# nianticlabs/simplerecon

Hardware: AMD Instinct MI355X
Metric: depth frames/sec (640x480, 7 src views, 64 planes) (higher is better)
Workload: dtype f32

## Files before the change

### include/simplerecon_hip.h

```cpp
#ifndef SIMPLERECON_HIP_H_
#define SIMPLERECON_HIP_H_

#include <stddef.h>
#include <stdint.h>

#ifdef __cplusplus
extern "C" {
#endif

#define SR_OK 0
#define SR_ERR_INVALID_ARGUMENT 1
#define SR_ERR_UNSUPPORTED 2
#define SR_ERR_WORKSPACE_TOO_SMALL 3
#define SR_ERR_HIP_BASE 1000

enum {
  SR_OPT_MLP_SPLIT = 0, SR_OPT_WINO_SPLIT, SR_OPT_WINO_XCD, SR_OPT_WINO_NT, SR_OPT_WINO_KSPLIT, SR_OPT_CONV_WINO,
  SR_OPT_CONV_TILE, SR_OPT_CONV_KSPLIT, SR_OPT_PW_NT, SR_OPT_PW_KS, SR_OPT_PT_CFG, SR_OPT_PT_KS, SR_OPT_DOT_LDS,
  SR_OPT_DOT_LDS_G, SR_OPT_DOT_LDS_CULL, SR_OPT_DOT_LDS_CAP, SR_OPT_UPSAMPLE_QUAD, SR_OPT_POOL_STREAM,
  SR_OPT_MLP_TILE,
  SR_OPT_COUNT
};
int sr_option_count(void);
const char* sr_option_name(int id);
int sr_option_id(const char* name);
int sr_option_get(int id, int* value);
int sr_option_set(int id, int value, int* previous );
int sr_option_default(int id, int* value);

int sr_abi_version(void);

const char* sr_target_arch(void);


size_t sr_volume_workspace_bytes(int B, int K, int C, int h, int w);

int sr_volume_prepare(const float* src, const float* K_src, const float* T_src_cur,
                      const float* T_cur_src, int B, int K, int C, int h, int w, void* workspace,
                      size_t workspace_bytes, void* stream);

int sr_dot_volume_sweep(const float* cur, const float* invK_cur, const float* planes, int64_t ps_b,
                        int64_t ps_d, int64_t ps_y, int64_t ps_x, int B, int K, int C, int h, int w,
                        int D, float* out_cv, int64_t cv_sb, int64_t cv_sd, int64_t cv_sp,
                        float* out_lowest, uint8_t* out_mask, void* workspace,
                        size_t workspace_bytes, void* stream);

int sr_conv3x3_wino_io_nhwc_fwd(const void* in, int64_t in_batch_stride, int in_pix_stride, const float* packed_u,
                                const float* bias, const void* residual, int64_t res_batch_stride, int res_pix_stride,
                                void* out, int64_t out_batch_stride, int out_pix_stride, int B, int H, int W, int Cin,
                                int Cout, float leaky_slope, int io_dtype, void* stream);
int sr_pw_conv_io_nhwc_fwd(const void* in, int64_t in_batch_stride, int in_pix_stride, const float* packed_w,
                           const float* bias, const void* residual, int64_t res_batch_stride, int res_pix_stride, void* out,
                           int64_t out_batch_stride, int out_pix_stride, int B, int HW, int Cin, int Cout, float act_code,
                           int io_dtype, void* stream);

size_t sr_pw_conv_tiled_workspace_bytes(int M, int Cin, int Cout);
int sr_pw_conv_tiled_plan(int M, int Cin, int Cout, int can_split, int* cfg, int* ks);
int sr_pw_conv_tiled_nhwc_fwd(const float* in, int in_pix_stride, const float* packed_w, const float* bias,
                              const float* gate, const float* residual, int res_pix_stride, float* out,
                              int out_pix_stride, int M, int HW, int Cin, int Cout, float act_code, void* workspace,
                              size_t workspace_bytes, void* stream);
int sr_pw_conv_supported(int Cin, int Cout);
int sr_pw_conv_plan(int B, int HW, int Cin, int Cout, int* nt, int* ks);
int sr_pw_conv_nhwc_fwd(const float* in, int64_t in_batch_stride, int in_pix_stride, const float* packed_w,
                        const float* bias, const float* gate, const float* residual, int64_t res_batch_stride,
                        int res_pix_stride, float* out, int64_t out_batch_stride, int out_pix_stride, int B, int HW,
                        int Cin, int Cout, float act_code, void* stream);

int sr_backproject_fwd(const float* depth, const float* invK, float* out_points, int B, int h, int w, void* stream);
int sr_project3d_fwd(const float* points, const float* K, const float* T, float* out, int B, int N, float eps,
                     void* stream);
int sr_backproject_bwd(const float* grad_points, const float* invK, float* grad_depth, int B, int h, int w, void* stream);
int sr_project3d_bwd(const float* grad_out, const float* points, const float* K, const float* T, float* grad_points, int B,
// ... 508 lines not shown
```

### simplerecon_amd/csrc/sr_common.h

```cpp
#pragma once
#include <hip/hip_runtime.h>
#include <stdint.h>

#include "simplerecon_hip.h"

#define SR_GEOM_STRIDE 20

#define SR_WAVE 64

int sr_opt(int id);

int sr_device_cus();

hipError_t sr_allow_lds(const void* kernel, size_t bytes);

enum SrKernel { SR_K_NONE = 0, SR_K_CONV, SR_K_WINO, SR_K_WINO_SPLIT, SR_K_WINO4, SR_K_PW, SR_K_PW_TILED, SR_K_STEM, SR_K_C1S,
                SR_K_T16 };
struct SrLaunchNote { int kernel, a, b, c, d, e, f; int64_t m, n, k; };
void sr_note_launch(const SrLaunchNote& note);

int sr_wgrad_reduce_launch(const float* part, float* d_weight, int Cout, int Cin, int taps, int ci_blocks, int per, int blocks,
                           hipStream_t stream);
int sr_bias_partial_reduce_launch(const float* partial, int blocks, int C, float* d_bias, hipStream_t stream);

static inline int sr_hip_rc(hipError_t e) { return e == hipSuccess ? SR_OK : SR_ERR_HIP_BASE + (int)e; }

static inline size_t sr_align_up(size_t v, size_t a) { return (v + a - 1) / a * a; }

struct SrPlanes {
  const float* ptr;
  int64_t sb, sd, sy, sx;
};

struct SrVolumeOut {
  float* cv;
  int64_t sb, sd, sp;
  float* lowest;
  uint8_t* mask;
};

struct SrSample {
  float zp;
  float pix_x, pix_y;
  float w_nw, w_ne, w_sw, w_se;
  int o_nw, o_ne, o_sw, o_se;
  bool any_tap;
};

typedef float sr_f2v __attribute__((ext_vector_type(2)));
typedef float f32x16 __attribute__((ext_vector_type(16)));

__device__ __forceinline__ void sr_bilinear_taps(float ix, float iy, int h, int w, float& fx0, float& fy0, float& w_nw,
                                                 float& w_ne, float& w_sw, float& w_se, bool& any_tap) {
#pragma clang fp contract(off)
  const sr_f2v ixy = {ix, iy};
  fx0 = floorf(ix);
  fy0 = floorf(iy);
  const sr_f2v f0 = {fx0, fy0};
  const sr_f2v f1 = f0 + 1.0f;
  const float fx1 = f1.x, fy1 = f1.y;
  const float wm = (float)(w - 1), hm = (float)(h - 1);
  const bool vx0 = (fx0 >= 0.0f) & (fx0 <= wm), vx1 = (fx1 >= 0.0f) & (fx1 <= wm);
  const bool vy0 = (fy0 >= 0.0f) & (fy0 <= hm), vy1 = (fy1 >= 0.0f) & (fy1 <= hm);
  const sr_f2v a1 = f1 - ixy, a0 = ixy - f0;
  const sr_f2v wtop = sr_f2v{a1.x, a0.x} * a1.y;
  const sr_f2v wbot = sr_f2v{a1.x, a0.x} * a0.y;
  w_nw = (vx0 & vy0) ? wtop.x : 0.0f;
  w_ne = (vx1 & vy0) ? wtop.y : 0.0f;
  w_sw = (vx0 & vy1) ? wbot.x : 0.0f;
  w_se = (vx1 & vy1) ? wbot.y : 0.0f;
  any_tap = (vx0 | vx1) & (vy0 | vy1);
}
__device__ __forceinline__ void sr_bilinear_taps(float ix, float iy, int h, int w, float& fx0, float& fy0, float& w_nw,
                                                 float& w_ne, float& w_sw, float& w_se) {
  bool any_tap;
  sr_bilinear_taps(ix, iy, h, w, fx0, fy0, w_nw, w_ne, w_sw, w_se, any_tap);
}

struct SrSampleXY {
  float zp, pix_x, pix_y;
// ... 114 lines not shown
__device__ __forceinline__ SrDotLane sr_dot_lane(const SrDotParams& p, int grp, int S) {
  SrDotLane l;
  l.lane = threadIdx.x & 63;
  l.grp = grp;
  l.S = S;
  l.b = blockIdx.y;
  l.N = p.h * p.w;
  l.tile = blockIdx.x;
  {
    const int nwg = gridDim.x, q = nwg >> 3, r = nwg & 7, xcd = l.tile & 7, idx = l.tile >> 3;
    l.tile = (xcd < r ? xcd * (q + 1) : r * (q + 1) + (xcd - r) * q) + idx;
  }
  l.pix = l.tile * 64 + l.lane;
  l.active = l.pix < l.N;
  l.pc = l.active ? l.pix : l.N - 1;
  l.y = l.pc / p.w;
  l.x = l.pc - l.y * p.w;
  const int per = (p.D + l.S - 1) / l.S;
  l.j0 = l.grp * per;
  l.j1 = min(p.D, l.j0 + per);
  return l;
}
__device__ __forceinline__ void sr_argmax_step(float cost, float d, float& best, float& best_d, bool& have) {
  if (!have || cost > best || (cost != cost && best == best)) { best = cost; best_d = d; have = true; }
}
__device__ __forceinline__ void sr_dot_store_lowest(const SrDotParams& p, const SrDotLane& l, float* smem, float best,
                                                    float best_d, bool have) {
  if (p.out.lowest) {
    if (gridDim.z > 1) {
    } else if (l.S == 1) {
      if (l.active) p.out.lowest[(size_t)l.b * l.N + l.pix] = best_d;
    } else {
      float* s_best = smem;
      float* s_d = smem + l.S * 64;
      float* s_have = smem + 2 * l.S * 64;
      s_best[l.grp * 64 + l.lane] = best;
      s_d[l.grp * 64 + l.lane] = best_d;
      s_have[l.grp * 64 + l.lane] = have ? 1.0f : 0.0f;
      __syncthreads();
      if (l.grp == 0 && l.active) {
        float bb = best, bd = best_d;
        for (int g = 1; g < l.S; ++g)
          if (s_have[g * 64 + l.lane] != 0.0f &&
              (s_best[g * 64 + l.lane] > bb || (s_best[g * 64 + l.lane] != s_best[g * 64 + l.lane] && bb == bb))) {
            bb = s_best[g * 64 + l.lane];
            bd = s_d[g * 64 + l.lane];
          }
        p.out.lowest[(size_t)l.b * l.N + l.pix] = bd;
      }
    }
  }
}

static inline float* sr_ws_geom(void* workspace) { return (float*)sr_align_up((size_t)workspace, 256); }
static inline float* sr_ws_src_nhwc(void* workspace, int B, int K) {
  return (float*)((char*)sr_ws_geom(workspace) + sr_align_up((size_t)B * K * SR_GEOM_STRIDE * sizeof(float), 256));
}

static inline size_t sr_ws_nhwc_bytes(int B, int K, int C, int h, int w) {
  return sr_align_up((size_t)B * K * h * w * C * sizeof(float), 256);
}
static inline unsigned long long* sr_ws_keys(void* workspace, int B, int K, int C, int h, int w) {
  return (unsigned long long*)((char*)sr_ws_src_nhwc(workspace, B, K) + sr_ws_nhwc_bytes(B, K, C, h, w));
}

int sr_launch_dot_volume_lds(const SrDotParams& p, unsigned long long* keys, hipStream_t stream);
int sr_launch_geom(const float* K_src, const float* T_src_cur, const float* T_cur_src, float* geom,
                   int n, hipStream_t stream);
int sr_launch_argmax_planes(const float* cv, int64_t sb, int64_t sd, int64_t sp, SrPlanes planes, int B, int h, int w,
                            int D, float* lowest, hipStream_t stream);
int sr_launch_splitk_reduce(const float* part, int ksplit, int64_t part_stride, const float* bias, const float* res,
                            int64_t res_sb, int res_sp, float* out, int64_t out_sb, int out_sp, int B, int HW, int Cout,
                            float slope, hipStream_t stream);
int sr_launch_unpack_nhwc(const float* src_nhwc, float* dst_nchw, int images, int C, int npix, hipStream_t stream);
int sr_launch_pack_nhwc(const float* src_nchw, float* dst_nhwc, int images, int C, int npix,
                        hipStream_t stream);
```

### simplerecon_amd/csrc/sr_dot_volume.hip

```cpp
#include <stdlib.h>

#include "sr_common.h"


__global__ void sr_geom_kernel(const float* __restrict__ K_src, const float* __restrict__ T_src_cur,
                               const float* __restrict__ T_cur_src, float* __restrict__ geom, int n) {
#pragma clang fp contract(off)
  const int i = blockIdx.x * blockDim.x + threadIdx.x;
  if (i >= n) return;
  const float* Km = K_src + 16 * (size_t)i;
  const float* T = T_src_cur + 16 * (size_t)i;
  float* g = geom + SR_GEOM_STRIDE * (size_t)i;
  for (int r = 0; r < 3; ++r)
    for (int c = 0; c < 4; ++c) {
      float s = 0.0f;
      for (int k = 0; k < 4; ++k) s += Km[r * 4 + k] * T[k * 4 + c];
      g[r * 4 + c] = s;
    }
  float t0 = 0.f, t1 = 0.f, t2 = 0.f, dist = 0.f, rm = 0.f, tm = 0.f;
  if (T_cur_src) {
    const float* Tc = T_cur_src + 16 * (size_t)i;
    t0 = Tc[3]; t1 = Tc[7]; t2 = Tc[11];
    const float tr = (Tc[0] + Tc[5]) + Tc[10];
    const float trc = tr > 3.0f ? 3.0f : tr;
    rm = sqrtf(2.0f * (1.0f - trc / 3.0f));
    tm = sqrtf((t0 * t0 + t1 * t1) + t2 * t2);
    dist = sqrtf(tm * tm + rm * rm);
  }
  g[12] = t0; g[13] = t1; g[14] = t2; g[15] = dist; g[16] = rm; g[17] = tm; g[18] = 0.f; g[19] = 0.f;
}

int sr_launch_geom(const float* K_src, const float* T_src_cur, const float* T_cur_src, float* geom,
                   int n, hipStream_t stream) {
  if (n == 0) return SR_OK;
  hipLaunchKernelGGL(sr_geom_kernel, dim3((n + 63) / 64), dim3(64), 0, stream, K_src, T_src_cur, T_cur_src,
                     geom, n);
  return sr_hip_rc(hipGetLastError());
}

template <int C>
__global__ __launch_bounds__(256) void sr_pack_nhwc_kernel(const float* __restrict__ src,
                                                           float* __restrict__ dst, int npix) {
  __shared__ float tile[64][C + 1];
  const int img = blockIdx.y;
  const int p0 = blockIdx.x * 64;
  const float* s = src + (size_t)img * C * npix;
  float* d = dst + (size_t)img * npix * C;
  for (int e = threadIdx.x; e < 64 * C; e += 256) {
    const int c = e >> 6, p = e & 63;
    tile[p][c] = (p0 + p < npix) ? s[(size_t)c * npix + p0 + p] : 0.0f;
  }
  __syncthreads();
  for (int e = threadIdx.x; e < 64 * C; e += 256) {
    const int p = e / C, c = e - p * C;
    if (p0 + p < npix) d[(size_t)(p0 + p) * C + c] = tile[p][c];
  }
}

int sr_launch_pack_nhwc(const float* src_nchw, float* dst_nhwc, int images, int C, int npix,
                        hipStream_t stream) {
  if (images == 0 || npix == 0) return SR_OK;
// ... 130 lines not shown
#pragma unroll 1
    for (int k = 0; k < p.K; ++k) {
      SrSample s;
      sr_project_sample(geom_b + k * SR_GEOM_STRIDE, X0, X1, X2, p.h, p.w, p.inv_w, p.inv_h, s);
      const bool front = s.zp > 0.0f;
      any_depth |= front;
      any_bounds |= sr_in_bounds(s, p.h, p.w);
      const float w_nw = front ? s.w_nw : 0.0f, w_ne = front ? s.w_ne : 0.0f;
      const float w_sw = front ? s.w_sw : 0.0f, w_se = front ? s.w_se : 0.0f;
      const float* img = src_b + (size_t)k * N * C + 4 * quad;
#pragma unroll
      for (int r = 0; r < 4; ++r) {
        const int sl = 16 * r + slot;
        const int o_nw = __shfl(s.o_nw, sl), o_ne = __shfl(s.o_ne, sl), o_sw = __shfl(s.o_sw, sl), o_se = __shfl(s.o_se, sl);
        const float a_nw = __shfl(w_nw, sl), a_ne = __shfl(w_ne, sl), a_sw = __shfl(w_sw, sl), a_se = __shfl(w_se, sl);
        const float4 t_nw = *reinterpret_cast<const float4*>(img + (size_t)o_nw * C);
        const float4 t_ne = *reinterpret_cast<const float4*>(img + (size_t)o_ne * C);
        const float4 t_sw = *reinterpret_cast<const float4*>(img + (size_t)o_sw * C);
        const float4 t_se = *reinterpret_cast<const float4*>(img + (size_t)o_se * C);
        const sr_f2 cl = {curq[r].x, curq[r].y}, ch = {curq[r].z, curq[r].w};
        const sr_f2 wnw = {a_nw, a_nw}, wne = {a_ne, a_ne}, wsw = {a_sw, a_sw}, wse = {a_se, a_se};
        sr_f2 lo = wnw * sr_f2{t_nw.x, t_nw.y}, hi = wnw * sr_f2{t_nw.z, t_nw.w};
        lo = __builtin_elementwise_fma(wne, sr_f2{t_ne.x, t_ne.y}, lo);
        hi = __builtin_elementwise_fma(wne, sr_f2{t_ne.z, t_ne.w}, hi);
        lo = __builtin_elementwise_fma(wsw, sr_f2{t_sw.x, t_sw.y}, lo);
        hi = __builtin_elementwise_fma(wsw, sr_f2{t_sw.z, t_sw.w}, hi);
        lo = __builtin_elementwise_fma(wse, sr_f2{t_se.x, t_se.y}, lo);
        hi = __builtin_elementwise_fma(wse, sr_f2{t_se.z, t_se.w}, hi);
        const sr_f2 pr = __builtin_elementwise_fma(hi, ch, lo * cl);
        costr[r] += pr.x + pr.y;
      }
    }
    float cost = 0.0f;
#pragma unroll
    for (int r = 0; r < 4; ++r) {
      const float v = __shfl(sr_quad_sum(costr[r]), gather_lane);
      cost = (lane >> 4) == r ? v : cost;
    }
    if (active) out[j * p.out.sd] = cost;
    sr_argmax_step(cost, d, best, best_d, have);
    if (j == p.D - 1 && p.out.mask && active)
      p.out.mask[(size_t)b * N + pix] = (uint8_t)(any_depth && any_bounds);
  }

  sr_dot_store_lowest(p, l, smem, best, best_d, have);
}


extern "C" int sr_abi_version(void) { return 4; }
extern "C" const char* sr_target_arch(void) { return "gfx950"; }

extern "C" size_t sr_volume_workspace_bytes(int B, int K, int C, int h, int w) {
  if (B < 0 || K < 0 || C < 0 || h < 0 || w < 0) return 0;
  const size_t geom = sr_align_up((size_t)B * K * SR_GEOM_STRIDE * sizeof(float), 256);
  const size_t nhwc = sr_ws_nhwc_bytes(B, K, C, h, w);
  const size_t keys = sr_align_up((size_t)B * h * w * sizeof(unsigned long long), 256);
  return geom + nhwc + keys + 256;
}

static int sr_pick_plane_split(int B, int N, int D) {
  const long tiles = (long)B * ((N + 63) / 64);
  int S = 1;
  while (S < 16 && tiles * S < 256L * 16 && S * 2 <= D) S *= 2;
  return S;
}

extern "C" int sr_volume_prepare(const float* src, const float* K_src, const float* T_src_cur,
                                 const float* T_cur_src, int B, int K, int C, int h, int w, void* workspace,
                                 size_t workspace_bytes, void* stream_) {
  if (B < 0 || K <= 0 || C <= 0 || h <= 0 || w <= 0) return SR_ERR_INVALID_ARGUMENT;
  if (B == 0) return SR_OK;
  if (!src || !K_src || !T_src_cur || !workspace) return SR_ERR_INVALID_ARGUMENT;
  if (C % 4 != 0 || C > 32) return SR_ERR_UNSUPPORTED;
  if (workspace_bytes < sr_volume_workspace_bytes(B, K, C, h, w)) return SR_ERR_WORKSPACE_TOO_SMALL;
  hipStream_t stream = (hipStream_t)stream_;
  int rc = sr_launch_geom(K_src, T_src_cur, T_cur_src, sr_ws_geom(workspace), B * K, stream);
  if (rc) return rc;
  return sr_launch_pack_nhwc(src, sr_ws_src_nhwc(workspace, B, K), B * K, C, h * w, stream);
}

extern "C" int sr_dot_volume_sweep(const float* cur, const float* invK_cur, const float* planes, int64_t ps_b,
                                   int64_t ps_d, int64_t ps_y, int64_t ps_x, int B, int K, int C, int h, int w,
                                   int D, float* out_cv, int64_t cv_sb, int64_t cv_sd, int64_t cv_sp,
                                   float* out_lowest, uint8_t* out_mask, void* workspace,
                                   size_t workspace_bytes, void* stream_) {
  if (B < 0 || K <= 0 || C <= 0 || h <= 0 || w <= 0 || D <= 0) return SR_ERR_INVALID_ARGUMENT;
  if (B == 0) return SR_OK;
  if (!cur || !invK_cur || !planes || !out_cv || !workspace) return SR_ERR_INVALID_ARGUMENT;
  if (C % 4 != 0 || C > 32) return SR_ERR_UNSUPPORTED;
  if (workspace_bytes < sr_volume_workspace_bytes(B, K, C, h, w)) return SR_ERR_WORKSPACE_TOO_SMALL;
  hipStream_t stream = (hipStream_t)stream_;
  const int N = h * w;

  SrDotParams p;
  p.cur = cur; p.src_nhwc = sr_ws_src_nhwc(workspace, B, K); p.invK = invK_cur; p.geom = sr_ws_geom(workspace);
  p.planes = {planes, ps_b, ps_d, ps_y, ps_x};
  p.out = {out_cv, cv_sb, cv_sd, cv_sp, out_lowest, out_mask};
  p.B = B; p.K = K; p.h = h; p.w = w; p.D = D;
  p.inv_w = (float)(1.0 / (double)w);
  p.inv_h = (float)(1.0 / (double)h);

  if (C == 16) {
    const int use_lds = sr_opt(SR_OPT_DOT_LDS);
    if (use_lds) {
      const int rc = sr_launch_dot_volume_lds(p, sr_ws_keys(workspace, B, K, C, h, w), stream);
      if (rc != SR_ERR_UNSUPPORTED) return rc;
    }
// ... 108 lines not shown
```

### simplerecon_amd/csrc/sr_mlp_volume.hip

```cpp
#include <stdlib.h>
#include <string.h>

#include "sr_buffer.h"
#include "sr_view.h"

#define SR_HID 128
#define SR_VIEW_SLOTS 24
#define SR_INV_FIXED 20
#define SR_PLANE_CHUNK 8

static inline int sr_mlp_steps_var(int K) { return (SR_VIEW_SLOTS / 2) * K; }
static inline int sr_mlp_steps_inv(int K) { return (SR_INV_FIXED + 3 * K + 1) / 2; }
static inline int sr_mlp_steps1(int K) { return sr_mlp_steps_var(K) + sr_mlp_steps_inv(K); }
#define SR_MLP_STEPS2 65

static inline size_t sr_mlp_packed_floats(int K) { return (size_t)(sr_mlp_steps1(K) + SR_MLP_STEPS2) * 256 + 128 + 4; }

#define SR_MLP_COLUMN_OFFSETS(K, C)                                                                    \
  const int o_cur = (K) * (C), o_mask = o_cur + (C), o_z = o_mask + (K), o_d = o_z + (K), o_dot = o_d + 1; \
  const int o_ang = o_dot + (K), o_cray = o_ang + (K), o_sray = o_cray + 3, o_pd = o_sray + 3 * (K);  \
  const int o_rm = o_pd + (K), o_tm = o_rm + (K);
__device__ __forceinline__ int sr_mlp_var_col(int K, int C, int k, int s) {
  SR_MLP_COLUMN_OFFSETS(K, C)
  (void)o_cur; (void)o_cray; (void)o_pd; (void)o_rm; (void)o_tm;
  if (s < 16) return k * C + s;
  if (s == 16) return o_mask + k;
  if (s == 17) return o_z + k;
  if (s == 18) return o_ang + k;
  if (s < 22) return o_sray + 3 * k + (s - 19);
  if (s == 22) return o_dot + k;
  return (k == 0) ? o_d : -1;
}
__device__ __forceinline__ int sr_mlp_inv_col(int K, int C, int u) {
  SR_MLP_COLUMN_OFFSETS(K, C)
  (void)o_mask; (void)o_z; (void)o_d; (void)o_dot; (void)o_ang; (void)o_sray;
  if (u < 16) return o_cur + u;
  if (u < 19) return o_cray + (u - 16);
  if (u == 19) return -2;
  if (u >= SR_INV_FIXED + 3 * K) return -1;
  const int k = (u - SR_INV_FIXED) / 3, i = (u - SR_INV_FIXED) - 3 * k;
  return (i == 0 ? o_pd : (i == 1 ? o_rm : o_tm)) + k;
}

__global__ void sr_mlp_pack_kernel(const float* __restrict__ W1, const float* __restrict__ b1,
                                   const float* __restrict__ W2, const float* __restrict__ b2,
                                   const float* __restrict__ W3, const float* __restrict__ b3,
                                   float* __restrict__ packed, int K, int C) {
  const int steps_var = (SR_VIEW_SLOTS / 2) * K;
  const int steps1 = steps_var + (SR_INV_FIXED + 3 * K + 1) / 2;
  const int Cin = C * (K + 1) + 10 * K + 4;
  const int total = (steps1 + SR_MLP_STEPS2) * 256 + 128 + 1;
  for (int e = blockIdx.x * blockDim.x + threadIdx.x; e < total; e += gridDim.x * blockDim.x) {
    float v = 0.0f;
    if (e < steps1 * 256) {
      const int t = e >> 8, lane = (e >> 2) & 63, mt = e & 3;
      const int row = 32 * mt + (lane & 31);
      int col;
      if (t < steps_var) {
        const int slot = 2 * t + (lane >> 5);
        const int k = slot / SR_VIEW_SLOTS;
        col = sr_mlp_var_col(K, C, k, slot - k * SR_VIEW_SLOTS);
      } else {
        col = sr_mlp_inv_col(K, C, 2 * (t - steps_var) + (lane >> 5));
      }
      v = (col >= 0) ? W1[(size_t)row * Cin + col] : (col == -2 ? b1[row] : 0.0f);
    } else if (e < (steps1 + SR_MLP_STEPS2) * 256) {
      const int e2 = e - steps1 * 256;
      const int t = e2 >> 8, lane = (e2 >> 2) & 63, mt = e2 & 3;
      const int row = 32 * mt + (lane & 31);
      if (t < 64) {
        const int m = t >> 4, r = t & 15;
        const int f = 32 * m + (r & 3) + 8 * (r >> 2) + 4 * (lane >> 5);
        v = W2[(size_t)row * SR_HID + f];
      } else {
        v = (lane < 32) ? b2[row] : 0.0f;
      }
    } else if (e < (steps1 + SR_MLP_STEPS2) * 256 + 128) {
      const int i = e - (steps1 + SR_MLP_STEPS2) * 256;
      const int half = i >> 6, mt = (i >> 4) & 3, r = i & 15;
      v = W3[32 * mt + (r & 3) + 8 * (r >> 2) + 4 * half];
    } else {
      v = b3[0];
    }
    packed[e] = v;
  }
}


struct SrMlpParams {
  const float* cur;
  const float* src_nhwc;
  const float* invK;
  const float* geom;
  const float* packed;
  SrPlanes planes;
  SrVolumeOut out;
  int B, K, h, w, D;
  int tiles;
  int tiles_x;
  int th_log2, tw_log2;
  int chunk, chunks;
  int cur_nhwc;
  int vec_store;
  float inv_w, inv_h, slope;
};

__device__ __forceinline__ bool sr_mlp_lane_pixel(const SrMlpParams& p, int tile, int lane, int& y, int& x) {
  if (p.tiles_x) {
    const int ty = tile / p.tiles_x, tx = tile - ty * p.tiles_x;
    const int ly = (ty << p.th_log2) + (lane >> p.tw_log2);
    const int lx = (tx << p.tw_log2) + (lane & ((1 << p.tw_log2) - 1));
    y = min(ly, p.h - 1);
    x = min(lx, p.w - 1);
    return ly < p.h && lx < p.w;
  }
  const int N = p.h * p.w, pix = tile * 64 + lane;
  const int pc = min(pix, N - 1);
  y = pc / p.w;
  x = pc - y * p.w;
  return pix < N;
}

__device__ __forceinline__ void sr_swap_halves(float fa, float fb, float& bP, float& bQ) {
  auto r = __builtin_amdgcn_permlane32_swap(__float_as_uint(fa), __float_as_uint(fb), false, false);
  bP = __uint_as_float(r[0]);
  bQ = __uint_as_float(r[1]);
}

#define SR_MFMA(a, b, c) __builtin_amdgcn_mfma_f32_32x32x2f32((a), (b), (c), 0, 0, 0)

__device__ __forceinline__ void sr_l1_step(f32x16 (&acc)[2][4], const float4 wA, float fa, float fb) {
  float bP, bQ;
  sr_swap_halves(fa, fb, bP, bQ);
  acc[0][0] = SR_MFMA(wA.x, bP, acc[0][0]);
  acc[1][0] = SR_MFMA(wA.x, bQ, acc[1][0]);
  acc[0][1] = SR_MFMA(wA.y, bP, acc[0][1]);
  acc[1][1] = SR_MFMA(wA.y, bQ, acc[1][1]);
  acc[0][2] = SR_MFMA(wA.z, bP, acc[0][2]);
  acc[1][2] = SR_MFMA(wA.z, bQ, acc[1][2]);
  acc[0][3] = SR_MFMA(wA.w, bP, acc[0][3]);
  acc[1][3] = SR_MFMA(wA.w, bQ, acc[1][3]);
}

__device__ __forceinline__ void sr_l1_step_init(f32x16 (&acc)[2][4], const f32x16 (&hc)[2][4], const float4 wA,
                                                float fa, float fb) {
  float bP, bQ;
  sr_swap_halves(fa, fb, bP, bQ);
  acc[0][0] = SR_MFMA(wA.x, bP, hc[0][0]);
  acc[1][0] = SR_MFMA(wA.x, bQ, hc[1][0]);
  acc[0][1] = SR_MFMA(wA.y, bP, hc[0][1]);
  acc[1][1] = SR_MFMA(wA.y, bQ, hc[1][1]);
  acc[0][2] = SR_MFMA(wA.z, bP, hc[0][2]);
  acc[1][2] = SR_MFMA(wA.z, bQ, hc[1][2]);
  acc[0][3] = SR_MFMA(wA.w, bP, hc[0][3]);
  acc[1][3] = SR_MFMA(wA.w, bQ, hc[1][3]);
}

__device__ __forceinline__ int sr_opaque(bool flag) {
  int v = __builtin_amdgcn_readfirstlane((int)flag);
  asm volatile("" : "+s"(v));
  return v;
}

#define SR_LDS_W3_FLOATS 256


__device__ __forceinline__ void sr_mlp_cur_ray(float d0, float r0, float r1, float r2, float& cr0, float& cr1, float& cr2,
                                               float& crn0, float& crn1, float& crn2) {
#pragma clang fp contract(off)
  const float X0 = d0 * r0, X1 = d0 * r1, X2 = d0 * r2;
  const float cden = fmaxf(sqrtf((X0 * X0 + X1 * X1) + X2 * X2), 1e-12f);
  cr0 = X0 / cden; cr1 = X1 / cden; cr2 = X2 / cden;
  const float n1 = fmaxf(sqrtf((cr0 * cr0 + cr1 * cr1) + cr2 * cr2), 1e-5f);
  crn0 = cr0 / n1; crn1 = cr1 / n1; crn2 = cr2 / n1;
}

__device__ __forceinline__ void sr_mlp_load_taps(const float* img, const SrSample& smp, float4 (&taps)[16]) {
  const float4* t_nw = reinterpret_cast<const float4*>(img + (size_t)smp.o_nw * 16);
  const float4* t_ne = reinterpret_cast<const float4*>(img + (size_t)smp.o_ne * 16);
  const float4* t_sw = reinterpret_cast<const float4*>(img + (size_t)smp.o_sw * 16);
  const float4* t_se = reinterpret_cast<const float4*>(img + (size_t)smp.o_se * 16);
#pragma unroll
  for (int i = 0; i < 4; ++i) {
    taps[i] = t_nw[i]; taps[4 + i] = t_ne[i]; taps[8 + i] = t_sw[i]; taps[12 + i] = t_se[i];
  }
}

template <bool W1_LDS, bool W2_LDS>
__global__ __launch_bounds__(256, 1) void sr_mlp_volume_kernel(SrMlpParams p) {
  extern __shared__ __attribute__((aligned(16))) float lds[];
  constexpr int C = 16;
  constexpr int VS = SR_VIEW_SLOTS / 2;
  const int lane = threadIdx.x & 63;
  const int steps_var = VS * p.K;
  const int steps1 = steps_var + (SR_INV_FIXED + 3 * p.K + 1) / 2;
  const float4* gW1 = reinterpret_cast<const float4*>(p.packed);
  const float4* gW1inv = gW1 + (size_t)steps_var * 64;
  const float4* gW2 = gW1 + (size_t)steps1 * 64;
  const float* gW3 = p.packed + (size_t)(steps1 + SR_MLP_STEPS2) * 256;

  for (int i = threadIdx.x; i < 129; i += blockDim.x) lds[i] = gW3[i];
  constexpr int W2_FLOATS = W2_LDS ? SR_MLP_STEPS2 * 256 : 0;
  if (W2_LDS) {
    float4* l4 = reinterpret_cast<float4*>(lds + SR_LDS_W3_FLOATS);
    for (int i = threadIdx.x; i < SR_MLP_STEPS2 * 64; i += blockDim.x) l4[i] = gW2[i];
  }
  if (W1_LDS) {
    float4* l4 = reinterpret_cast<float4*>(lds + SR_LDS_W3_FLOATS + W2_FLOATS);
    for (int i = threadIdx.x; i < steps_var * 64; i += blockDim.x) l4[i] = gW1[i];
  }
  __syncthreads();
  const float4* W1p = W1_LDS ? reinterpret_cast<const float4*>(lds + SR_LDS_W3_FLOATS + W2_FLOATS) : gW1;

  const int N = p.h * p.w;
  const long nunits = (long)p.B * p.tiles * p.chunks;
  constexpr int WPB = 4;
  const int wid = __builtin_amdgcn_readfirstlane(threadIdx.x >> 6);
  long wave0 = (long)blockIdx.x * WPB + wid;
  long nwaves = (long)gridDim.x * WPB;
  long unit_end = nunits;
  if ((gridDim.x & 7) == 0) {
    const long u8 = (nunits + 7) / 8;
    const int xcd = blockIdx.x & 7;
    nwaves = (long)(gridDim.x >> 3) * WPB;
    wave0 = xcd * u8 + (long)(blockIdx.x >> 3) * WPB + wid;
    unit_end = min(nunits, (xcd + 1) * u8);
  }
  const int half = lane >> 5;

  const int rot = (int)max(1L, nwaves / p.chunks);
  for (long unit = wave0; unit < unit_end; unit += nwaves) {
    const long tb = unit / p.chunks;
    const int chunk = (int)((unit % p.chunks + tb / rot) % p.chunks);
    const int tile = (int)(tb % p.tiles);
    const int b = (int)(tb / p.tiles);
    const int j0 = chunk * p.chunk, j1 = min(p.D, j0 + p.chunk);
    int y, x;
    const bool in_image = sr_mlp_lane_pixel(p, tile, lane, y, x);
    const int pc = y * p.w + x;
    const int pix = in_image ? pc : -1;
    const bool active = pix >= 0;
    const float* plane_ptr = p.planes.ptr + b * p.planes.sb + y * p.planes.sy + x * p.planes.sx;
    const float* geom_b = p.geom + (size_t)b * p.K * SR_GEOM_STRIDE;
    const float* src_b = p.src_nhwc + (size_t)b * p.K * N * C;

    float cur[C];
    if (p.cur_nhwc) {
      const float4* c4 = reinterpret_cast<const float4*>(p.cur + ((size_t)b * N + pc) * C);
#pragma unroll
      for (int i = 0; i < C / 4; ++i) {
        const float4 v = c4[i];
        cur[4 * i] = v.x; cur[4 * i + 1] = v.y; cur[4 * i + 2] = v.z; cur[4 * i + 3] = v.w;
      }
    } else {
#pragma unroll
      for (int c = 0; c < C; ++c) cur[c] = p.cur[((size_t)b * C + c) * N + pc];
    }

    float r0, r1, r2;
    sr_pixel_ray(p.invK + 16 * (size_t)b, x, y, r0, r1, r2);
    float cr0, cr1, cr2, crn0, crn1, crn2;
    sr_mlp_cur_ray(plane_ptr[0], r0, r1, r2, cr0, cr1, cr2, crn0, crn1, crn2);

    f32x16 hc[2][4];
#pragma unroll
    for (int g = 0; g < 2; ++g)
#pragma unroll
      for (int m = 0; m < 4; ++m)
#pragma unroll
        for (int r = 0; r < 16; ++r) hc[g][m][r] = 0.0f;
    {
      const float4* wi = gW1inv + lane;
#pragma unroll
      for (int t = 0; t < 8; ++t) sr_l1_step(hc, wi[t * 64], cur[2 * t], cur[2 * t + 1]);
      sr_l1_step(hc, wi[8 * 64], cr0, cr1);
      sr_l1_step(hc, wi[9 * 64], cr2, 1.0f);
      const int npose = 3 * p.K;
#pragma unroll 1
      for (int u = 0; u < npose; u += 2) {
        const int ka = u / 3, ia = u - 3 * ka, kb = (u + 1) / 3, ib = (u + 1) - 3 * kb;
        const float fa = geom_b[ka * SR_GEOM_STRIDE + 15 + ia];
        const float fb = (u + 1 < npose) ? geom_b[kb * SR_GEOM_STRIDE + 15 + ib] : 0.0f;
        sr_l1_step(hc, wi[(size_t)(10 + (u >> 1)) * 64], fa, fb);
      }
    }

    SrSample smp;
    float4 taps[16];
    float X0, X1, X2, d;
// ... 195 lines not shown
        acc2[1][3] = SR_MFMA(wA.w, one, acc2[1][3]);
      }

      const float4* w3 = reinterpret_cast<const float4*>(lds + half * 64);
      sr_f2v oPQ = {0.0f, 0.0f};
      const sr_f2v slope2 = {p.slope, p.slope};
#pragma unroll
      for (int m = 0; m < 4; ++m)
#pragma unroll
        for (int q = 0; q < 4; ++q) {
          const float4 wv = w3[m * 4 + q];
          const float wr[4] = {wv.x, wv.y, wv.z, wv.w};
#pragma unroll
          for (int i = 0; i < 4; ++i) {
            const sr_f2v h2 = {acc2[0][m][4 * q + i], acc2[1][m][4 * q + i]};
            const sr_f2v s2 = slope2 * h2;
            oPQ = __builtin_elementwise_fma(sr_f2v{wr[i], wr[i]}, sr_f2v{sr_vmax(h2.x, s2.x), sr_vmax(h2.y, s2.y)}, oPQ);
          }
        }
      float oP = oPQ.x, oQ = oPQ.y;
      oP += __shfl_xor(oP, 32);
      oQ += __shfl_xor(oQ, 32);
      const float cost = (half ? oQ : oP) + lds[128];

      if (p.vec_store) {
        if (CST_LDS) lds[cst_base + (j - j0) * 64 + lane] = cost;
        else {
#pragma unroll
          for (int q = 0; q < SR_PLANE_CHUNK; ++q) cst[q] = (j - j0 == q) ? cost : cst[q];
        }
      }
      if (active) {
        if (!p.vec_store) p.out.cv[b * p.out.sb + j * p.out.sd + (int64_t)pix * p.out.sp] = cost;
        if (j == p.D - 1 && p.out.mask) p.out.mask[(size_t)b * N + pix] = (uint8_t)(any_depth && any_bounds);
      }
    }
    if (p.vec_store && active) {
      float* row = p.out.cv + b * p.out.sb + (int64_t)pix * p.out.sp + j0;
      if (CST_LDS) {
#pragma unroll
        for (int q = 0; q < SR_PLANE_CHUNK; ++q) cst[q] = lds[cst_base + q * 64 + lane];
      }
#pragma unroll
      for (int q = 0; q < SR_PLANE_CHUNK; q += 4) {
        if (j0 + q + 4 <= j1) *reinterpret_cast<float4*>(row + q) = make_float4(cst[q], cst[q + 1], cst[q + 2], cst[q + 3]);
        else {
#pragma unroll
          for (int i = 0; i < 4; ++i)
            if (j0 + q + i < j1) row[q + i] = cst[q + i];
        }
      }
    }
  }
}


template <int FMT> struct SrSplitFmt;
template <> struct SrSplitFmt<1> {
  typedef __bf16 e2 __attribute__((ext_vector_type(2)));
  typedef __bf16 e8 __attribute__((ext_vector_type(8)));
  static __device__ __forceinline__ void split(float a, float b, unsigned& hi, unsigned& lo) {
    const sr_f2v v = {a, b};
    hi = __builtin_bit_cast(unsigned, __builtin_convertvector(v, e2));
    const sr_f2v v0 = {__uint_as_float(hi << 16), __uint_as_float(hi & 0xffff0000u)};
    lo = __builtin_bit_cast(unsigned, __builtin_convertvector(v - v0, e2));
  }
  static __device__ __forceinline__ f32x16 mfma(sr_u4 a, sr_u4 b, f32x16 c) {
    return __builtin_amdgcn_mfma_f32_32x32x16_bf16(__builtin_bit_cast(e8, a), __builtin_bit_cast(e8, b), c, 0, 0, 0);
  }
};
template <> struct SrSplitFmt<2> {
  typedef _Float16 e2 __attribute__((ext_vector_type(2)));
  typedef _Float16 e8 __attribute__((ext_vector_type(8)));
  static __device__ __forceinline__ void split(float a, float b, unsigned& hi, unsigned& lo) {
    const sr_f2v v = {a, b};
    const e2 h = __builtin_convertvector(v, e2);
    hi = __builtin_bit_cast(unsigned, h);
    lo = __builtin_bit_cast(unsigned, __builtin_convertvector(v - __builtin_convertvector(h, sr_f2v), e2));
  }
  static __device__ __forceinline__ f32x16 mfma(sr_u4 a, sr_u4 b, f32x16 c) {
    return __builtin_amdgcn_mfma_f32_32x32x16_f16(__builtin_bit_cast(e8, a), __builtin_bit_cast(e8, b), c, 0, 0, 0);
  }
};

#define SR_SPL_TAB 512
#define SR_SPL_W2_WORDS 16384
#define SR_SPL_VIEW_WORDS 3072

template <int FMT>
__global__ void sr_mlp_pack_split_kernel(const float* __restrict__ W1, const float* __restrict__ b1,
                                         const float* __restrict__ W2, const float* __restrict__ b2,
                                         const float* __restrict__ W3, const float* __restrict__ b3,
                                         float* __restrict__ packed, int K, int C) {
  typedef SrSplitFmt<FMT> S;
  const int steps_var = (SR_VIEW_SLOTS / 2) * K;
  const int steps_inv = (SR_INV_FIXED + 3 * K + 1) / 2;
  const int steps1 = steps_var + steps_inv;
  const int Cin = C * (K + 1) + 10 * K + 4;
  unsigned* pk = reinterpret_cast<unsigned*>(packed);
  auto put = [&](size_t word, int piece, float wa, float wb) {
    unsigned hi, lo;
    S::split(wa, wb, hi, lo);
    pk[word] = piece ? lo : hi;
  };
  const int total = (steps1 + SR_MLP_STEPS2) * 256 + 128 + 1;
  for (int e = blockIdx.x * blockDim.x + threadIdx.x; e < total; e += gridDim.x * blockDim.x) {
// ... 329 lines not shown
      const int64_t tiles = (int64_t)((h + t - 1) / t) * ((w + 64 / t - 1) / (64 / t));
      if (100 * tiles <= 101 * flat) { *th = t; *tw = 64 / t; break; }
    }
  }
  return SR_OK;
}

static float* sr_ws_packed(void* workspace, int B, int K, int C, int h, int w) {
  return (float*)sr_align_up((size_t)workspace + sr_volume_workspace_bytes(B, K, C, h, w), 256);
}

static int sr_mlp_volume_sweep_reserved(const float* cur, const float* src_nhwc, const float* invK_cur,
                                        const float* planes, int64_t ps_b,
                                        int64_t ps_d, int64_t ps_y, int64_t ps_x, float leaky_slope, int B, int K,
                                        int C, int h, int w, int D, float* out_cv, int64_t cv_sb, int64_t cv_sd,
                                        int64_t cv_sp, float* out_lowest, uint8_t* out_mask, int reserve_cus,
                                        void* workspace, size_t workspace_bytes, void* stream_) {
  if (B < 0 || K <= 0 || C <= 0 || h <= 0 || w <= 0 || D <= 0) return SR_ERR_INVALID_ARGUMENT;
  if (B == 0) return SR_OK;
  if (!cur || !invK_cur || !planes || !out_cv || !workspace) return SR_ERR_INVALID_ARGUMENT;
  if (C != 16) return SR_ERR_UNSUPPORTED;
  if (!(leaky_slope > 0.0f && leaky_slope < 1.0f)) return SR_ERR_UNSUPPORTED;
  if (workspace_bytes < sr_mlp_volume_workspace_bytes(B, K, C, h, w, SR_HID)) return SR_ERR_WORKSPACE_TOO_SMALL;
  hipStream_t stream = (hipStream_t)stream_;
  const int N = h * w;

  SrMlpParams p;
  p.cur = cur; p.src_nhwc = src_nhwc ? src_nhwc : sr_ws_src_nhwc(workspace, B, K); p.cur_nhwc = src_nhwc != nullptr;
  p.invK = invK_cur; p.geom = sr_ws_geom(workspace);
  p.packed = sr_ws_packed(workspace, B, K, C, h, w);
  p.planes = {planes, ps_b, ps_d, ps_y, ps_x};
  p.out = {out_cv, cv_sb, cv_sd, cv_sp, out_lowest, out_mask};
  p.B = B; p.K = K; p.h = h; p.w = w; p.D = D;
  int th, tw;
  if (sr_mlp_volume_tile_shape(h, w, &th, &tw)) return SR_ERR_INVALID_ARGUMENT;
  p.th_log2 = __builtin_ctz(th); p.tw_log2 = __builtin_ctz(tw);
  p.tiles_x = th == 1 ? 0 : (w + tw - 1) / tw;
  p.tiles = th == 1 ? (N + 63) / 64 : p.tiles_x * ((h + th - 1) / th);
  p.inv_w = (float)(1.0 / (double)w);
  p.inv_h = (float)(1.0 / (double)h);
  p.slope = leaky_slope;

  int cus = sr_device_cus();
  if (reserve_cus > 0 && cus - reserve_cus >= 8) cus -= reserve_cus;
  const long waves = 4L * cus;
  double best_cost = 1e30;
  int best = 1;
  for (int c = SR_PLANE_CHUNK; c >= 1; c >>= 1) {
    const long units = (long)B * p.tiles * ((D + c - 1) / c);
    const long rounds = (units + waves - 1) / waves;
    const double cost = (double)rounds * (c * 1192.0 + 168.0);
    if (cost < best_cost) { best_cost = cost; best = c; }
  }
  p.chunk = best;
  p.chunks = (D + best - 1) / best;
  p.vec_store = (cv_sd == 1) && (p.chunk % 4 == 0) && sr_rows_aligned(out_cv, cv_sb, cv_sp, 15, 4);
  const long nunits = (long)B * p.tiles * p.chunks;
  const int blocks = (int)((nunits + 3) / 4 < cus ? (nunits + 3) / 4 : cus);
  const size_t w3_bytes = SR_LDS_W3_FLOATS * sizeof(float);
  const size_t w1_bytes = (size_t)sr_mlp_steps_var(K) * 1024;
  const size_t w2_bytes = (size_t)SR_MLP_STEPS2 * 1024;
  const size_t lds_max = 160 * 1024;
  const int split = sr_mlp_split_mode();
  if (split < 0) return SR_ERR_INVALID_ARGUMENT;
  if (split) {
    if (p.cur_nhwc) return SR_ERR_UNSUPPORTED;
    const size_t bytes = ((size_t)SR_SPL_TAB + SR_SPL_W2_WORDS + (size_t)K * SR_SPL_VIEW_WORDS) * 4;
    if (bytes > lds_max) return SR_ERR_UNSUPPORTED;
    const void* fn = split == 1 ? (const void*)sr_mlp_volume_split_kernel<1> : (const void*)sr_mlp_volume_split_kernel<2>;
    if (hipError_t e = sr_allow_lds(fn, bytes)) return sr_hip_rc(e);
    if (split == 1) hipLaunchKernelGGL((sr_mlp_volume_split_kernel<1>), dim3(blocks), dim3(256), bytes, stream, p);
    else hipLaunchKernelGGL((sr_mlp_volume_split_kernel<2>), dim3(blocks), dim3(256), bytes, stream, p);
    int rc = sr_hip_rc(hipGetLastError());
    if (rc) return rc;
    if (out_lowest) rc = sr_launch_argmax_planes(out_cv, cv_sb, cv_sd, cv_sp, p.planes, B, h, w, D, out_lowest, stream);
    return rc;
  }
#define SR_MLP_LAUNCH(L1, L2, BYTES)                                                                              \
  {                                                                                                               \
           \
    if (hipError_t e = sr_allow_lds((const void*)sr_mlp_volume_kernel<L1, L2>, (BYTES))) return sr_hip_rc(e);     \
    hipLaunchKernelGGL((sr_mlp_volume_kernel<L1, L2>), dim3(blocks), dim3(256), (BYTES), stream, p);              \
  }
  if (w1_bytes + w2_bytes + w3_bytes <= lds_max) SR_MLP_LAUNCH(true, true, w1_bytes + w2_bytes + w3_bytes)
  else if (w1_bytes + w3_bytes <= lds_max) SR_MLP_LAUNCH(true, false, w1_bytes + w3_bytes)
  else SR_MLP_LAUNCH(false, true, w2_bytes + w3_bytes + 4 * SR_PLANE_CHUNK * 64 * sizeof(float))
#undef SR_MLP_LAUNCH
  int rc = sr_hip_rc(hipGetLastError());
  if (rc) return rc;
  if (out_lowest) rc = sr_launch_argmax_planes(out_cv, cv_sb, cv_sd, cv_sp, p.planes, B, h, w, D, out_lowest, stream);
  return rc;
}

extern "C" int sr_mlp_volume_sweep(const float* cur, const float* invK_cur, const float* planes, int64_t ps_b,
                                   int64_t ps_d, int64_t ps_y, int64_t ps_x, float leaky_slope, int B, int K,
                                   int C, int h, int w, int D, float* out_cv, int64_t cv_sb, int64_t cv_sd,
                                   int64_t cv_sp, float* out_lowest, uint8_t* out_mask, void* workspace,
                                   size_t workspace_bytes, void* stream_) {
  return sr_mlp_volume_sweep_reserved(cur, nullptr, invK_cur, planes, ps_b, ps_d, ps_y, ps_x, leaky_slope, B, K, C, h, w, D,
                                      out_cv, cv_sb, cv_sd, cv_sp, out_lowest, out_mask, 0, workspace, workspace_bytes, stream_);
}

int sr_launch_argmax_planes(const float* cv, int64_t sb, int64_t sd, int64_t sp, SrPlanes planes, int B, int h, int w,
                            int D, float* lowest, hipStream_t stream) {
  hipLaunchKernelGGL(sr_argmax_planes_kernel, dim3((h * w + 63) / 64, B), dim3(64), 0, stream, cv, sb, sd, sp,
                     planes, h, w, D, lowest);
  return sr_hip_rc(hipGetLastError());
}

extern "C" int sr_mlp_pack_weights(const float* W1, const float* b1, const float* W2, const float* b2,
                                   const float* W3, const float* b3, int hidden, int B, int K, int C, int h, int w,
                                   void* workspace, size_t workspace_bytes, void* stream_) {
  if (!W1 || !b1 || !W2 || !b2 || !W3 || !b3 || !workspace || K <= 0) return SR_ERR_INVALID_ARGUMENT;
  if (hidden != SR_HID || C != 16) return SR_ERR_UNSUPPORTED;
  if (workspace_bytes < sr_mlp_volume_workspace_bytes(B, K, C, h, w, hidden)) return SR_ERR_WORKSPACE_TOO_SMALL;
  const int split = sr_mlp_split_mode();
  if (split < 0) return SR_ERR_INVALID_ARGUMENT;
  float* packed = sr_ws_packed(workspace, B, K, C, h, w);
  if (split == 1) hipLaunchKernelGGL((sr_mlp_pack_split_kernel<1>), dim3(64), dim3(256), 0, (hipStream_t)stream_, W1, b1, W2, b2, W3, b3, packed, K, C);
  else if (split == 2) hipLaunchKernelGGL((sr_mlp_pack_split_kernel<2>), dim3(64), dim3(256), 0, (hipStream_t)stream_, W1, b1, W2, b2, W3, b3, packed, K, C);
  else hipLaunchKernelGGL(sr_mlp_pack_kernel, dim3(64), dim3(256), 0, (hipStream_t)stream_, W1, b1, W2, b2, W3, b3, packed, K, C);
  return sr_hip_rc(hipGetLastError());
}

static int sr_mlp_volume_run(bool nhwc, const float* cur, const float* src, const float* K_src, const float* T_src_cur,
                             const float* T_cur_src, const float* invK_cur, const float* planes, int64_t ps_b,
                             int64_t ps_d, int64_t ps_y, int64_t ps_x, const float* W1, const float* b1,
                             const float* W2, const float* b2, const float* W3, const float* b3, int hidden,
                             float leaky_slope, int B, int K, int C, int h, int w, int D, float* out_cv,
                             int64_t cv_sb, int64_t cv_sd, int64_t cv_sp, float* out_lowest, uint8_t* out_mask,
                             int reserve_cus, void* workspace, size_t workspace_bytes, void* stream_) {
  if (B < 0 || K <= 0 || C <= 0 || h <= 0 || w <= 0 || D <= 0 || reserve_cus < 0) return SR_ERR_INVALID_ARGUMENT;
  if (B == 0) return SR_OK;
  if (!T_cur_src) return SR_ERR_INVALID_ARGUMENT;
  if (nhwc) {
    if (!cur || !src || !K_src || !T_src_cur || !workspace) return SR_ERR_INVALID_ARGUMENT;
    if (((size_t)cur | (size_t)src) & 15) return SR_ERR_INVALID_ARGUMENT;
  }
  if (hidden != SR_HID || C != 16) return SR_ERR_UNSUPPORTED;
  if (nhwc) {
// ... 39 lines not shown
```

### simplerecon_amd/csrc/sr_options.hip

```cpp
#include <atomic>
#include <map>
#include <mutex>
#include <utility>
#include <stdio.h>
#include <stdlib.h>
#include <string.h>

#include "sr_common.h"

namespace {

struct OptDef { const char* name; int dflt; int kind; };
const OptDef kDefs[SR_OPT_COUNT] = {
    {"SR_MLP_SPLIT", 0, 1},       {"SR_WINO_SPLIT", 0, 1},     {"SR_WINO_XCD", 1, 0},        {"SR_WINO_NT", 0, 0},
    {"SR_WINO_KSPLIT", 0, 0},     {"SR_CONV_WINO", 1, 0},      {"SR_CONV_TILE", 0, 0},       {"SR_CONV_KSPLIT", 1, 0},
    {"SR_PW_NT", 0, 0},           {"SR_PW_KS", 0, 0},          {"SR_PT_CFG", -1, 0},         {"SR_PT_KS", 0, 0},
    {"SR_DOT_LDS", 1, 0},         {"SR_DOT_LDS_G", 0, 0},      {"SR_DOT_LDS_CULL", 1, 0},    {"SR_DOT_LDS_CAP", 634, 0},
    {"SR_UPSAMPLE_QUAD", 1, 0},   {"SR_POOL_STREAM", 1, 0},    {"SR_MLP_TILE", 0, 2},
};
std::atomic<int> g_val[SR_OPT_COUNT];
std::once_flag g_once;

int parse(const OptDef& d, const char* e) {
  if (d.kind == 1) {
    if (!e || !*e || !strcmp(e, "0") || !strcmp(e, "off") || !strcmp(e, "fp32")) return 0;
    if (!strcmp(e, "bf16")) return 1;
    if (!strcmp(e, "f16") || !strcmp(e, "fp16")) return 2;
    return -1;
  }
  if (d.kind == 2) {
    static const char* const names[] = {"auto", "flat", "2x32", "4x16", "8x8"};
    if (!e || !*e) return d.dflt;
    for (int i = 0; i < 5; ++i)
      if (!strcmp(e, names[i])) return i;
    return -1;
  }
  return (e && *e) ? atoi(e) : d.dflt;
}

void init() {
  for (int i = 0; i < SR_OPT_COUNT; ++i) {
    const char* e = getenv(kDefs[i].name);
    g_val[i].store(e ? parse(kDefs[i], e) : kDefs[i].dflt, std::memory_order_relaxed);
  }
}

}

int sr_opt(int id) {
  std::call_once(g_once, init);
  return g_val[id].load(std::memory_order_relaxed);
}

extern "C" int sr_option_count(void) { return SR_OPT_COUNT; }

extern "C" const char* sr_option_name(int id) { return (id >= 0 && id < SR_OPT_COUNT) ? kDefs[id].name : nullptr; }

extern "C" int sr_option_id(const char* name) {
  if (!name) return -1;
  for (int i = 0; i < SR_OPT_COUNT; ++i)
    if (!strcmp(kDefs[i].name, name)) return i;
  return -1;
}

extern "C" int sr_option_get(int id, int* value) {
  if (id < 0 || id >= SR_OPT_COUNT || !value) return SR_ERR_INVALID_ARGUMENT;
  *value = sr_opt(id);
  return SR_OK;
}

extern "C" int sr_option_set(int id, int value, int* previous) {
// ... 64 lines not shown
```

Baseline: 328.3.

## Schedule MLP volume work units via per-XCD atomic queue with finer tail chunks

Replaces the static strided assignment of (tile, plane-chunk) units to waves in the MLP cost-volume kernel with a dynamic per-XCD atomic ticket queue. The last fraction of tiles (set by a tail shift) is split into half-size plane chunks so the tail is balanced better. Counters live in the geometry workspace, are zeroed by the geom kernel, and are reset by the last block to finish. This targets load imbalance and tail idle time, at the cost of one atomic per unit, a block-wide sync at exit, and a forced chunk size. Optional trace instrumentation is compiled in only under a macro.

```diff
diff --git a/include/simplerecon_hip.h b/include/simplerecon_hip.h
--- a/include/simplerecon_hip.h
+++ b/include/simplerecon_hip.h
@@ -18,7 +18,7 @@
   SR_OPT_MLP_SPLIT = 0, SR_OPT_WINO_SPLIT, SR_OPT_WINO_XCD, SR_OPT_WINO_NT, SR_OPT_WINO_KSPLIT, SR_OPT_CONV_WINO,
   SR_OPT_CONV_TILE, SR_OPT_CONV_KSPLIT, SR_OPT_PW_NT, SR_OPT_PW_KS, SR_OPT_PT_CFG, SR_OPT_PT_KS, SR_OPT_DOT_LDS,
   SR_OPT_DOT_LDS_G, SR_OPT_DOT_LDS_CULL, SR_OPT_DOT_LDS_CAP, SR_OPT_UPSAMPLE_QUAD, SR_OPT_POOL_STREAM,
-  SR_OPT_MLP_TILE,
+  SR_OPT_MLP_TILE, SR_OPT_MLP_QUEUE,
   SR_OPT_COUNT
 };
 int sr_option_count(void);
diff --git a/simplerecon_amd/csrc/sr_common.h b/simplerecon_amd/csrc/sr_common.h
--- a/simplerecon_amd/csrc/sr_common.h
+++ b/simplerecon_amd/csrc/sr_common.h
@@ -25,7 +25,7 @@
 
 static inline int sr_hip_rc(hipError_t e) { return e == hipSuccess ? SR_OK : SR_ERR_HIP_BASE + (int)e; }
 
-static inline size_t sr_align_up(size_t v, size_t a) { return (v + a - 1) / a * a; }
+__host__ __device__ static inline size_t sr_align_up(size_t v, size_t a) { return (v + a - 1) / a * a; }
 
 struct SrPlanes {
   const float* ptr;
@@ -246,9 +246,15 @@
   }
 }
 
+#define SR_WS_COUNTERS 16
+__host__ __device__ static inline size_t sr_ws_counters_offset(size_t n) { return sr_align_up(n * SR_GEOM_STRIDE * sizeof(float), 64); }
+static inline size_t sr_ws_geom_bytes(size_t n) { return sr_align_up(sr_ws_counters_offset(n) + SR_WS_COUNTERS * 4, 256); }
 static inline float* sr_ws_geom(void* workspace) { return (float*)sr_align_up((size_t)workspace, 256); }
+static inline unsigned* sr_ws_counters(void* workspace, int B, int K) {
+  return (unsigned*)((char*)sr_ws_geom(workspace) + sr_ws_counters_offset((size_t)B * K));
+}
 static inline float* sr_ws_src_nhwc(void* workspace, int B, int K) {
-  return (float*)((char*)sr_ws_geom(workspace) + sr_align_up((size_t)B * K * SR_GEOM_STRIDE * sizeof(float), 256));
+  return (float*)((char*)sr_ws_geom(workspace) + sr_ws_geom_bytes((size_t)B * K));
 }
 
 static inline size_t sr_ws_nhwc_bytes(int B, int K, int C, int h, int w) {
diff --git a/simplerecon_amd/csrc/sr_dot_volume.hip b/simplerecon_amd/csrc/sr_dot_volume.hip
--- a/simplerecon_amd/csrc/sr_dot_volume.hip
+++ b/simplerecon_amd/csrc/sr_dot_volume.hip
@@ -7,6 +7,7 @@
                                const float* __restrict__ T_cur_src, float* __restrict__ geom, int n) {
 #pragma clang fp contract(off)
   const int i = blockIdx.x * blockDim.x + threadIdx.x;
+  if (i < SR_WS_COUNTERS) reinterpret_cast<unsigned*>(geom)[sr_ws_counters_offset((size_t)n) / 4 + i] = 0u;
   if (i >= n) return;
   const float* Km = K_src + 16 * (size_t)i;
   const float* T = T_src_cur + 16 * (size_t)i;
@@ -243,7 +244,7 @@
 
 extern "C" size_t sr_volume_workspace_bytes(int B, int K, int C, int h, int w) {
   if (B < 0 || K < 0 || C < 0 || h < 0 || w < 0) return 0;
-  const size_t geom = sr_align_up((size_t)B * K * SR_GEOM_STRIDE * sizeof(float), 256);
+  const size_t geom = sr_ws_geom_bytes((size_t)B * K);
   const size_t nhwc = sr_ws_nhwc_bytes(B, K, C, h, w);
   const size_t keys = sr_align_up((size_t)B * h * w * sizeof(unsigned long long), 256);
   return geom + nhwc + keys + 256;
diff --git a/simplerecon_amd/csrc/sr_mlp_volume.hip b/simplerecon_amd/csrc/sr_mlp_volume.hip
--- a/simplerecon_amd/csrc/sr_mlp_volume.hip
+++ b/simplerecon_amd/csrc/sr_mlp_volume.hip
@@ -1,3 +1,4 @@
+#include <stdio.h>
 #include <stdlib.h>
 #include <string.h>
 
@@ -103,7 +104,16 @@
   int cur_nhwc;
   int vec_store;
   float inv_w, inv_h, slope;
+  unsigned* queue;
+  int tail_shift;
+#ifdef SR_MLP_TRACE
+  unsigned long long* trace;
+#endif
 };
+#define SR_MLP_TR_WORDS 8
+#ifndef SR_MLP_TAIL_SHIFT
+#define SR_MLP_TAIL_SHIFT 4
+#endif
 
 __device__ __forceinline__ bool sr_mlp_lane_pixel(const SrMlpParams& p, int tile, int lane, int& y, int& x) {
   if (p.tiles_x) {
@@ -192,6 +202,9 @@
   constexpr int C = 16;
   constexpr int VS = SR_VIEW_SLOTS / 2;
   const int lane = threadIdx.x & 63;
+#ifdef SR_MLP_TRACE
+  const unsigned long long tr_t0 = __builtin_amdgcn_s_memtime(), tr_r0 = __builtin_amdgcn_s_memrealtime();
+#endif
   const int steps_var = VS * p.K;
   const int steps1 = steps_var + (SR_INV_FIXED + 3 * p.K + 1) / 2;
   const float4* gW1 = reinterpret_cast<const float4*>(p.packed);
@@ -213,28 +226,77 @@
   const float4* W1p = W1_LDS ? reinterpret_cast<const float4*>(lds + SR_LDS_W3_FLOATS + W2_FLOATS) : gW1;
 
   const int N = p.h * p.w;
-  const long nunits = (long)p.B * p.tiles * p.chunks;
   constexpr int WPB = 4;
   const int wid = __builtin_amdgcn_readfirstlane(threadIdx.x >> 6);
-  long wave0 = (long)blockIdx.x * WPB + wid;
-  long nwaves = (long)gridDim.x * WPB;
-  long unit_end = nunits;
-  if ((gridDim.x & 7) == 0) {
-    const long u8 = (nunits + 7) / 8;
-    const int xcd = blockIdx.x & 7;
-    nwaves = (long)(gridDim.x >> 3) * WPB;
-    wave0 = xcd * u8 + (long)(blockIdx.x >> 3) * WPB + wid;
-    unit_end = min(nunits, (xcd + 1) * u8);
-  }
   const int half = lane >> 5;
 
-  const int rot = (int)max(1L, nwaves / p.chunks);
-  for (long unit = wave0; unit < unit_end; unit += nwaves) {
-    const long tb = unit / p.chunks;
-    const int chunk = (int)((unit % p.chunks + tb / rot) % p.chunks);
+
+#ifdef SR_MLP_TRACE
+  unsigned long long* tr = p.trace + ((size_t)blockIdx.x * WPB + wid) * SR_MLP_TR_WORDS;
+  unsigned long long tr_units = 0;
+  if (lane == 0) {
+    tr[0] = tr_t0; tr[3] = tr_r0; tr[1] = __builtin_amdgcn_s_memtime();
+    tr[6] = ((unsigned long long)__builtin_amdgcn_s_getreg(20 | (0 << 6) | (3 << 11)) << 32) |
+            (unsigned long long)__builtin_amdgcn_s_getreg(4 | (0 << 6) | (31 << 11));
+  }
+#endif
+  for (int it = 0;; ++it) {
+    long tb;
+    int j0, j1;
+    unsigned z = 0;
+    asm volatile("" : "+s"(z));
+    const unsigned grid = gridDim.x + z;
+    const bool by_xcd = (grid & 7) == 0;
+    const unsigned xcd = by_xcd ? (blockIdx.x & 7) : 0;
+    if (p.queue) {
+      unsigned ticket = 0;
+      if (lane == 0) ticket = atomicAdd(p.queue + xcd, 1u);
+      const unsigned q = (unsigned)__builtin_amdgcn_readfirstlane((int)ticket);
+      unsigned q_tb0 = 0, q_ntb = (unsigned)(p.B * p.tiles);
+      if (by_xcd) {
+        const unsigned t8 = (q_ntb + 7) / 8;
+        q_tb0 = min(q_ntb, xcd * t8);
+        q_ntb = min(q_ntb, (xcd + 1) * t8) - q_tb0;
+      }
+      const unsigned q_half = (unsigned)p.chunk >> 1;
+      const unsigned q_chunks2 = q_half ? (p.D + q_half - 1) / q_half : 1;
+      const unsigned q_fine_tb = q_ntb >> p.tail_shift;
+      const unsigned q_coarse = (q_ntb - q_fine_tb) * p.chunks;
+      if (q >= q_coarse + q_fine_tb * q_chunks2) break;
+      if (q < q_coarse) {
+        tb = q_tb0 + q / (unsigned)p.chunks;
+        j0 = (int)(q % (unsigned)p.chunks) * p.chunk;
+        j1 = min(p.D, j0 + p.chunk);
+      } else {
+        const unsigned q2 = q - q_coarse;
+        tb = q_tb0 + (q_ntb - q_fine_tb) + q2 / q_chunks2;
+        j0 = (int)((q2 % q_chunks2) * q_half);
+        j1 = min(p.D, j0 + (int)q_half);
+      }
+    } else {
+      const long nunits = (long)p.B * p.tiles * p.chunks;
+      long wave0 = (long)blockIdx.x * WPB + wid;
+      long nwaves = (long)grid * WPB;
+      long unit_end = nunits;
+      if (by_xcd) {
+        const long u8 = (nunits + 7) / 8;
+        nwaves = (long)(grid >> 3) * WPB;
+        wave0 = xcd * u8 + (long)(blockIdx.x >> 3) * WPB + wid;
+        unit_end = min(nunits, (xcd + 1) * u8);
+      }
+      const int rot = (int)max(1L, nwaves / p.chunks);
+      const long unit = wave0 + it * nwaves;
+      if (unit >= unit_end) break;
+      tb = unit / p.chunks;
+      const int chunk = (int)((unit % p.chunks + tb / rot) % p.chunks);
+      j0 = chunk * p.chunk;
+      j1 = min(p.D, j0 + p.chunk);
+    }
+#ifdef SR_MLP_TRACE
+    ++tr_units;
+#endif
     const int tile = (int)(tb % p.tiles);
     const int b = (int)(tb / p.tiles);
-    const int j0 = chunk * p.chunk, j1 = min(p.D, j0 + p.chunk);
     int y, x;
     const bool in_image = sr_mlp_lane_pixel(p, tile, lane, y, x);
     const int pc = y * p.w + x;
@@ -536,6 +598,16 @@
       }
     }
   }
+#ifdef SR_MLP_TRACE
+  if (lane == 0) { tr[2] = __builtin_amdgcn_s_memtime(); tr[4] = __builtin_amdgcn_s_memrealtime(); tr[5] = tr_units; }
+#endif
+  if (p.queue) {
+    __syncthreads();
+    if (threadIdx.x == 0 && atomicAdd(p.queue + 8, 1u) == gridDim.x - 1) {
+#pragma unroll
+      for (int i = 0; i < 9; ++i) atomicExch(p.queue + i, 0u);
+    }
+  }
 }
 
 
@@ -971,6 +1043,12 @@
     const double cost = (double)rounds * (c * 1192.0 + 168.0);
     if (cost < best_cost) { best_cost = cost; best = c; }
   }
+  const int split = sr_mlp_split_mode();
+  if (split < 0) return SR_ERR_INVALID_ARGUMENT;
+  const bool queue = !split && sr_opt(SR_OPT_MLP_QUEUE) != 0 && (long)B * p.tiles < (1L << 27);
+  if (queue) best = SR_PLANE_CHUNK;
+  p.queue = queue ? sr_ws_counters(workspace, B, K) : nullptr;
+  p.tail_shift = (queue && best >= 8) ? SR_MLP_TAIL_SHIFT : 31;
   p.chunk = best;
   p.chunks = (D + best - 1) / best;
   p.vec_store = (cv_sd == 1) && (p.chunk % 4 == 0) && sr_rows_aligned(out_cv, cv_sb, cv_sp, 15, 4);
@@ -980,8 +1058,14 @@
   const size_t w1_bytes = (size_t)sr_mlp_steps_var(K) * 1024;
   const size_t w2_bytes = (size_t)SR_MLP_STEPS2 * 1024;
   const size_t lds_max = 160 * 1024;
-  const int split = sr_mlp_split_mode();
-  if (split < 0) return SR_ERR_INVALID_ARGUMENT;
+#ifdef SR_MLP_TRACE
+  static unsigned long long* trace_buf = nullptr;
+  const size_t trace_n = (size_t)blocks * 4 * SR_MLP_TR_WORDS;
+  if (!trace_buf) (void)hipMalloc((void**)&trace_buf, (size_t)4096 * SR_MLP_TR_WORDS * 8);
+  if (blocks > 1024) return SR_ERR_UNSUPPORTED;
+  (void)hipMemsetAsync(trace_buf, 0, trace_n * 8, stream);
+  p.trace = trace_buf;
+#endif
   if (split) {
     if (p.cur_nhwc) return SR_ERR_UNSUPPORTED;
     const size_t bytes = ((size_t)SR_SPL_TAB + SR_SPL_W2_WORDS + (size_t)K * SR_SPL_VIEW_WORDS) * 4;
@@ -1005,6 +1089,19 @@
   else if (w1_bytes + w3_bytes <= lds_max) SR_MLP_LAUNCH(true, false, w1_bytes + w3_bytes)
   else SR_MLP_LAUNCH(false, true, w2_bytes + w3_bytes + 4 * SR_PLANE_CHUNK * 64 * sizeof(float))
 #undef SR_MLP_LAUNCH
+#ifdef SR_MLP_TRACE
+  {
+    const char* path = getenv("SR_MLP_TRACE_FILE");
+    if (path && *path) {
+      (void)hipStreamSynchronize(stream);
+      unsigned long long* host = (unsigned long long*)malloc(trace_n * 8);
+      (void)hipMemcpy(host, trace_buf, trace_n * 8, hipMemcpyDeviceToHost);
+      FILE* f = fopen(path, "wb");
+      if (f) { int hdr[4] = {blocks * 4, SR_MLP_TR_WORDS, p.queue != nullptr, p.tail_shift}; fwrite(hdr, 4, 4, f); fwrite(host, 8, trace_n, f); fclose(f); }
+      free(host);
+    }
+  }
+#endif
   int rc = sr_hip_rc(hipGetLastError());
   if (rc) return rc;
   if (out_lowest) rc = sr_launch_argmax_planes(out_cv, cv_sb, cv_sd, cv_sp, p.planes, B, h, w, D, out_lowest, stream);
diff --git a/simplerecon_amd/csrc/sr_options.hip b/simplerecon_amd/csrc/sr_options.hip
--- a/simplerecon_amd/csrc/sr_options.hip
+++ b/simplerecon_amd/csrc/sr_options.hip
@@ -17,6 +17,7 @@
     {"SR_PW_NT", 0, 0},           {"SR_PW_KS", 0, 0},          {"SR_PT_CFG", -1, 0},         {"SR_PT_KS", 0, 0},
     {"SR_DOT_LDS", 1, 0},         {"SR_DOT_LDS_G", 0, 0},      {"SR_DOT_LDS_CULL", 1, 0},    {"SR_DOT_LDS_CAP", 634, 0},
     {"SR_UPSAMPLE_QUAD", 1, 0},   {"SR_POOL_STREAM", 1, 0},    {"SR_MLP_TILE", 0, 2},
+    {"SR_MLP_QUEUE", 1, 0},
 };
 std::atomic<int> g_val[SR_OPT_COUNT];
 std::once_flag g_once;
```

Measured after the change: 329.3, median of 6. About the same (+0.3%).
